# codex-storage/codex-storage-proofs-circuits

Hardware: AMD Instinct MI355X
Metric: Poseidon2-BN254 permutations/sec per GPU; full proof-input witnesses/sec (higher is better)
Workload: dtype u32x9 (29-bit limbs, Montgomery mod BN254 r)

## Files before the change

### codex-storage-proofs-circuits_amd/csrc/proof_many.cpp

```cpp
#include <hip/hip_runtime.h>

#include <algorithm>
#include <cstring>
#include <map>
#include <memory>
#include <string>
#include <vector>

#include "dataset_obj.hpp"
#include "proof_input_obj.hpp"
#include "trees.hpp"

using namespace cp2i;

namespace {

struct Req {
  cp2_dataset* ds = nullptr;
  uint64_t slot = 0;
  uint8_t entropy[32];
  size_t at = 0;
  size_t id = 0;
};

int refuse(cp2_ctx* ctx, size_t i, const std::string& why) {
  ctx->err = "request " + std::to_string(i) + ": " + why;
  return CP2_ERR_INVALID;
}

size_t depth_of(size_t n) { return layer_sizes_of(n).size() - 1; }

bool same_circuit(const cp2_config& a, const cp2_config& b) {
  return a.max_depth == b.max_depth && a.max_log2_nslots == b.max_log2_nslots && a.cell_size == b.cell_size && a.block_size == b.block_size &&
         a.n_samples == b.n_samples;
}

int validate(cp2_ctx* ctx, cp2_dataset* const* ds, const uint64_t* slot_idx, size_t n) {
  for (size_t i = 0; i < n; ++i) {
    const cp2_dataset* d = ds[i];
    if (!d) return refuse(ctx, i, "NULL dataset");
    if (d->ctx != ctx) return refuse(ctx, i, "its dataset belongs to another context");
    const cp2_config& c = d->cfg;
    if (!same_circuit(c, ds[0]->cfg))
      return refuse(ctx, i, "its circuit parameters (maxDepth, maxLog2NSlots, cellSize, blockSize, nSamples) differ from request 0's");
    const uint64_t s = slot_idx[i];
    if (s < d->first_slot || s - d->first_slot >= d->n_local)
      return refuse(ctx, i, "slot " + std::to_string(s) + " is not local to its dataset (slots " + std::to_string(d->first_slot) + " .. " +
                                std::to_string(d->first_slot + d->n_local - 1) + ")");
    if (!d->have_roots && !(d->first_slot == 0 && d->n_local == c.n_slots))
      return refuse(ctx, i, "its dataset has no dataset tree: not all of its slots are local and cp2_dataset_set_roots was never called");
    const std::string shape = proof_shape_refusal(c, config_slot_tree_depth(c), config_dataset_tree_depth(c));
    if (!shape.empty()) return refuse(ctx, i, shape);
    if (!d->trees && d->tree_mode == 2 && d->csizes.size() - 1 != depth_of(c.n_cells / (c.block_size / c.cell_size)))
      return refuse(ctx, i, "its compact layers do not match its configuration");
  }
  return CP2_OK;
}

int check_roots(cp2_ctx* ctx, cp2_dataset* const* ds, const uint64_t* slot_idx, size_t n) {
  std::vector<uint64_t> a(n);
  for (size_t i = 0; i < n; ++i)
    a[i] = (uint64_t)reinterpret_cast<uintptr_t>(dataset_roots_dev(ds[i])) + (slot_idx[i] - ds[i]->first_slot) * 32;
  std::vector<uint8_t> got(n * 32);
  DevBuf d_a, d_r;
  CP2_TRY(d_a.scratch(ctx, n * 8));
  CP2_TRY(d_r.scratch(ctx, n * 32));
  CP2_HIP(ctx, hipMemcpyAsync(d_a.p, a.data(), n * 8, hipMemcpyHostToDevice, ctx->stream));
  CP2_HIP(ctx, cp2k::launch_gather_addr(static_cast<const uint64_t*>(d_a.p), n, 32, d_r.p, ctx->stream));
  CP2_HIP(ctx, hipMemcpyAsync(got.data(), d_r.p, n * 32, hipMemcpyDeviceToHost, ctx->stream));
  CP2_HIP(ctx, hipStreamSynchronize(ctx->stream));
  for (size_t i = 0; i < n; ++i)
    if (std::memcmp(&got[i * 32], &ds[i]->dlayers[slot_idx[i] * 32], 32) != 0)
      return refuse(ctx, i, "the root its dataset tree holds for slot " + std::to_string(slot_idx[i]) +
                                " (cp2_dataset_set_roots) differs from the slot's built root");
  return CP2_OK;
}

int prepare(cp2_ctx* ctx, cp2_dataset* const* ds, const uint64_t* slot_idx, size_t n) {
  CP2_TRY(validate(ctx, ds, slot_idx, n));
  CP2_HIP(ctx, hipSetDevice(ctx->device));
  for (size_t i = 0; i < n; ++i)
    if (!ds[i]->have_roots) CP2_TRY(cp2_dataset_set_roots(ds[i], nullptr));
  return check_roots(ctx, ds, slot_idx, n);
}

std::string who(bool named, const Req* r) { return named ? "request " + std::to_string(r->id) + ": " : std::string(); }

int run_pass(cp2_ctx* ctx, const std::vector<const Req*>& rq, size_t n_rf, size_t n_rfile, size_t n_cf, bool named, cp2_proof_input** out) {
  const size_t n = rq.size(), nr = n_rf + n_rfile;
  const cp2_config& c0 = rq[0]->ds->cfg;
  const size_t ns = c0.n_samples, md = (size_t)c0.max_depth, cs = c0.cell_size, bs = c0.block_size, cpb = bs / cs;
  const size_t T = n * ns, R = nr * ns, C = T - R, RF = n_rf * ns, CF = n_cf * ns;
  auto store = std::make_shared<BatchStore>();
  if (T) {
    std::vector<cp2k::ManyReq> reqs(n);
    std::vector<cp2k::TreeGeom> geoms;
    std::map<std::string, uint32_t> geom_of;
    for (size_t j = 0; j < n; ++j) {
      const cp2_dataset* ds = rq[j]->ds;
      cp2k::ManyReq& q = reqs[j];
      std::memset(&q, 0, sizeof q);
      std::memcpy(q.entropy, rq[j]->entropy, 32);
      std::memcpy(q.slot_root, &ds->dlayers[rq[j]->slot * 32], 32);
      q.n_cells = ds->cfg.n_cells;
      q.cpb = cpb;
      if (j < nr) {
        cp2k::TreeGeom g;
        std::memset(&g, 0, sizeof g);
        trees_geom(ds->trees, &g);
        auto it = geom_of.emplace(std::string(reinterpret_cast<const char*>(&g), sizeof g), (uint32_t)geoms.size());
        if (it.second) geoms.push_back(g);
        q.geom = it.first->second;
        q.nodes = (uint64_t)reinterpret_cast<uintptr_t>(ds->trees->nodes.p);
        q.slot = rq[j]->slot - ds->first_slot;
      }
    }
    std::vector<uint64_t> blk(C), gen, cpaths, ctail, ccell;
    std::vector<uint8_t> checks(2 * C * 32);
    PinBuf h_blocks;
    const size_t rows = T * md + T + 2 * C;
    DevBuf d_req, d_geom, d_idx, d_blk, d_addr, d_rows, d_cells, d_gen, d_caddr;
    CP2_TRY(d_req.scratch(ctx, n * sizeof(cp2k::ManyReq)));
    CP2_TRY(d_geom.scratch(ctx, std::max<size_t>(1, geoms.size()) * sizeof(cp2k::TreeGeom)));
    CP2_TRY(d_idx.scratch(ctx, T * 8));
    CP2_TRY(d_blk.scratch(ctx, T * 8));
    CP2_TRY(d_addr.scratch(ctx, rows * 8));
    CP2_TRY(d_rows.scratch(ctx, rows * 32));
    CP2_TRY(d_cells.scratch(ctx, (C * cpb + T) * cs));
    CP2_TRY(store->idx.alloc(ctx, T * 8));
    CP2_TRY(store->paths.alloc(ctx, T * md * 32));
    CP2_TRY(store->leaves.alloc(ctx, T * 32));
    CP2_TRY(store->cells.alloc(ctx, T * cs));
    uint8_t* cells_out = d_cells.u8() + C * cpb * cs;
    uint64_t* addr = static_cast<uint64_t*>(d_addr.p);
    CP2_HIP(ctx, hipMemcpyAsync(d_req.p, reqs.data(), n * sizeof(cp2k::ManyReq), hipMemcpyHostToDevice, ctx->stream));
    if (!geoms.empty())
      CP2_HIP(ctx, hipMemcpyAsync(d_geom.p, geoms.data(), geoms.size() * sizeof(cp2k::TreeGeom), hipMemcpyHostToDevice, ctx->stream));
    CP2_HIP(ctx, cp2k::launch_sample_many(static_cast<const cp2k::ManyReq*>(d_req.p), static_cast<const cp2k::TreeGeom*>(d_geom.p), n,
                                          (uint32_t)ns, (uint32_t)md, static_cast<uint64_t*>(d_idx.p), static_cast<uint64_t*>(d_blk.p), addr,
                                          ctx->stream));
    CP2_HIP(ctx, hipMemcpyAsync(store->idx.p, d_idx.p, T * 8, hipMemcpyDeviceToHost, ctx->stream));
    if (C) CP2_HIP(ctx, hipMemcpyAsync(blk.data(), static_cast<uint64_t*>(d_blk.p) + R, C * 8, hipMemcpyDeviceToHost, ctx->stream));
    CP2_HIP(ctx, hipStreamSynchronize(ctx->stream));
    const uint64_t* idx = static_cast<const uint64_t*>(store->idx.p);

    gen.assign((CF + RF) * 2, 0);
    uint64_t* seeds = gen.data();
    uint64_t* firsts = seeds + CF + RF;
    for (size_t q = 0; q < CF; ++q) {
      const Req* r = rq[nr + q / ns];
      seeds[q] = cp2_slot_seed(r->ds->cfg.seed, r->slot);
      firsts[q] = blk[q] * cpb;
    }
    for (size_t p = 0; p < RF; ++p) {
      const Req* r = rq[p / ns];
      seeds[CF + p] = cp2_slot_seed(r->ds->cfg.seed, r->slot);
      firsts[CF + p] = idx[p];
    }
    if (CF + RF) {
      CP2_TRY(d_gen.scratch(ctx, gen.size() * 8));
      const uint64_t* dg = static_cast<const uint64_t*>(d_gen.p);
      CP2_HIP(ctx, hipMemcpyAsync(d_gen.p, gen.data(), gen.size() * 8, hipMemcpyHostToDevice, ctx->stream));
      CP2_HIP(ctx, cp2k::launch_gen_fake_cells_many(dg, dg + CF + RF, cpb, CF * cpb, cs, d_cells.p, ctx->stream));
      CP2_HIP(ctx, cp2k::launch_gen_fake_cells_many(dg + CF, dg + CF + RF + CF, 1, RF, cs, cells_out, ctx->stream));
    }
    if (C > CF) {
      const size_t n_req_file = (C - CF) / ns;
      CP2_TRY(h_blocks.alloc(ctx, (C - CF) * bs));
      std::vector<std::string> failed(fill_threads(ctx));
      on_threads(fill_threads(ctx), n_req_file, [&](int w, size_t k) {
        const size_t q0 = CF + k * ns;
        const Req* r = rq[nr + q0 / ns];
        const std::string fname = slot_file_name(r->ds->file_base, r->slot);
        size_t bad = 0;
        const int err = slot_file_read_list(fname, ns, [&](size_t) { return bs; }, [&](size_t c) { return blk[q0 + c] * bs; },
                                            [&](size_t c) { return h_blocks.u8() + (q0 - CF + c) * bs; }, &bad);
        if (err >= 0)
          failed[w] = who(named, r) + (err ? "block " + std::to_string(blk[q0 + bad]) + " of slot " : std::string("slot ")) + std::to_string(r->slot) +
                      ": " + slot_file_error(fname, err);
        return err < 0;
      });
      for (const auto& f : failed)
        if (!f.empty()) { ctx->err = f; return CP2_ERR_IO; }
      CP2_HIP(ctx, hipMemcpyAsync(d_cells.u8() + CF * bs, h_blocks.p, (C - CF) * bs, hipMemcpyHostToDevice, ctx->stream));
    }
    cp2_slot_trees* mini = nullptr;
    struct Mini { cp2_slot_trees*& t; ~Mini() { cp2_slot_trees_free(t); } } mini_guard{mini};
    if (C) {
      cpaths.assign(C * md, 0);
      ctail.assign(3 * C, 0);
      ccell.assign(C, 0);
      CP2_TRY(cp2_slot_trees_build_dev(ctx, d_cells.p, C, cs, bs, cpb, &mini));
      const size_t depth_b = depth_of(cpb);
      const uint64_t mb = (uint64_t)reinterpret_cast<uintptr_t>(mini->nodes.p);
      std::vector<uint64_t> rr(depth_b + 1);
      for (size_t q = 0; q < C; ++q) {
        const Req* r = rq[nr + q / ns];
        const cp2_dataset* ds = r->ds;
        const uint64_t ls = r->slot - ds->first_slot, cell = idx[R + q], b = blk[q], in_block = cell % cpb;
        const uint64_t kb = (uint64_t)reinterpret_cast<uintptr_t>(ds->compact.p);
        uint64_t* P = &cpaths[q * md];
        path_rows(mini, q, in_block, depth_b + 1, rr.data());
        for (size_t d = 0; d < depth_b; ++d) P[d] = rr[d] == NO_ROW ? 0 : mb + rr[d] * 32;
        uint64_t j = b, m = ds->cfg.n_cells / cpb;
        for (size_t d = 0; d + 1 < ds->csizes.size(); ++d) {
          const uint64_t sib = j ^ 1;
          P[depth_b + d] = sib < m ? kb + (ds->coff[d] + ls * ds->csizes[d] + sib) * 32 : 0;
          j >>= 1;
          m = (m + 1) >> 1;
        }
        ctail[q] = mb + (q * cpb + in_block) * 32;
        ctail[C + 2 * q] = kb + (ds->coff[0] + ls * ds->csizes[0] + b) * 32;
        ctail[C + 2 * q + 1] = mb + (mini->toff[0] + q) * 32;
        ccell[q] = (uint64_t)reinterpret_cast<uintptr_t>(d_cells.u8()) + (q * cpb + in_block) * cs;
      }
      CP2_TRY(d_caddr.scratch(ctx, C * 8));
      CP2_HIP(ctx, hipMemcpyAsync(addr + R * md, cpaths.data(), C * md * 8, hipMemcpyHostToDevice, ctx->stream));
      CP2_HIP(ctx, hipMemcpyAsync(addr + T * md + R, ctail.data(), 3 * C * 8, hipMemcpyHostToDevice, ctx->stream));
      CP2_HIP(ctx, hipMemcpyAsync(d_caddr.p, ccell.data(), C * 8, hipMemcpyHostToDevice, ctx->stream));
      CP2_HIP(ctx, cp2k::launch_gather_addr(static_cast<const uint64_t*>(d_caddr.p), C, cs, cells_out + R * cs, ctx->stream));
    }
    CP2_HIP(ctx, cp2k::launch_gather_addr(addr, rows, 32, d_rows.p, ctx->stream));
    CP2_HIP(ctx, hipMemcpyAsync(store->paths.p, d_rows.p, T * md * 32, hipMemcpyDeviceToHost, ctx->stream));
    CP2_HIP(ctx, hipMemcpyAsync(store->leaves.p, d_rows.u8() + T * md * 32, T * 32, hipMemcpyDeviceToHost, ctx->stream));
    if (C) CP2_HIP(ctx, hipMemcpyAsync(checks.data(), d_rows.u8() + (T * md + T) * 32, 2 * C * 32, hipMemcpyDeviceToHost, ctx->stream));
    CP2_HIP(ctx, hipMemcpyAsync(store->cells.p, cells_out, T * cs, hipMemcpyDeviceToHost, ctx->stream));
    CP2_HIP(ctx, hipStreamSynchronize(ctx->stream));
    for (size_t q = 0; q < C; ++q)
      if (std::memcmp(&checks[2 * q * 32], &checks[(2 * q + 1) * 32], 32) != 0) {
        const Req* r = rq[nr + q / ns];
        ctx->err = who(named, r) + "block " + std::to_string(blk[q]) + " of slot " + std::to_string(r->slot) +
                   " does not hash to its stored root (slot data changed since the build?)";
        return CP2_ERR_IO;
      }
    if (R > RF) {
      std::vector<std::string> failed(fill_threads(ctx));
      on_threads(fill_threads(ctx), n_rfile, [&](int w, size_t k) {
        const Req* r = rq[n_rf + k];
        const std::string fname = slot_file_name(r->ds->file_base, r->slot);
        const size_t p0 = (n_rf + k) * ns;
        const int err = slot_file_read_list(fname, ns, [&](size_t) { return cs; }, [&](size_t c) { return idx[p0 + c] * cs; },
                                            [&](size_t c) { return store->cells.u8() + (p0 + c) * cs; });
        if (err >= 0) failed[w] = who(named, r) + slot_file_error(fname, err);
        return err < 0;
      });
      for (const auto& f : failed)
        if (!f.empty()) { ctx->err = f; return CP2_ERR_IO; }
    }
  }
  std::vector<ProofItem> items(n);
  for (size_t j = 0; j < n; ++j) items[j] = {rq[j]->ds, rq[j]->slot, rq[j]->entropy, &out[rq[j]->at]};
  return proof_inputs_from_store(items.data(), n, store, store->cells.u8());
}

}

int cp2i::prove_requests(cp2_ctx* ctx, cp2_dataset* const* ds, const uint64_t* slot_idx, const uint8_t* entropies, size_t n, size_t at0,
                         bool named, cp2_proof_input** out) {
  for (size_t i = 0; i < n; ++i) out[i] = nullptr;
  if (n == 0) return CP2_OK;
  CP2_HIP(ctx, hipSetDevice(ctx->device));
  std::vector<Req> req(n);
  std::vector<const Req*> res_fake, res_file, cmp_fake, cmp_file, roots_only;
  for (size_t i = 0; i < n; ++i) {
    req[i].ds = ds[i];
    req[i].slot = slot_idx[i];
    req[i].at = i;
    req[i].id = at0 + i;
    canonical_felt(entropies + 32 * i, req[i].entropy);
    const cp2_dataset* d = ds[i];
    (d->trees ? (d->from_file ? res_file : res_fake) : d->tree_mode == 2 ? (d->from_file ? cmp_file : cmp_fake) : roots_only).push_back(&req[i]);
  }
  auto fail = [&](int st) {
    for (size_t i = 0; i < n; ++i) { cp2_proof_input_free(out[i]); out[i] = nullptr; }
    return st;
  };
  for (const Req* r : roots_only) {
    const int st = cp2_proof_inputs_generate_batch(r->ds, &r->slot, 1, r->entropy, &out[r->at]);
    if (st != CP2_OK) {
      ctx->err = who(named, r) + ctx->err;
      return fail(st);
    }
  }
  const cp2_config& c0 = ds[0]->cfg;
  const size_t per_req = std::max<size_t>(1, (size_t)c0.n_samples * c0.block_size);
  const size_t chunk = std::max<size_t>(1, ctx->stage_bytes / per_req);
  std::vector<const Req*> compact(cmp_fake);
  compact.insert(compact.end(), cmp_file.begin(), cmp_file.end());
  const size_t n_res = res_fake.size() + res_file.size();
  size_t c = 0;
  for (bool first = true; first ? n_res + compact.size() > 0 : c < compact.size(); first = false) {
    std::vector<const Req*> rq;
    if (first) {
      rq = res_fake;
      rq.insert(rq.end(), res_file.begin(), res_file.end());
    }
    const size_t c1 = std::min(compact.size(), c + chunk);
    rq.insert(rq.end(), compact.begin() + (long)c, compact.begin() + (long)c1);
    const size_t n_cf = c < cmp_fake.size() ? std::min(c1, cmp_fake.size()) - c : 0;
    const int st = run_pass(ctx, rq, first ? res_fake.size() : 0, first ? res_file.size() : 0, n_cf, named, out);
    if (st != CP2_OK) return fail(st);
    c = c1;
  }
  return CP2_OK;
}

extern "C" int cp2_proof_inputs_generate_many(cp2_ctx* ctx, cp2_dataset* const* ds, const uint64_t* slot_idx, const uint8_t* entropies, size_t n,
                                              cp2_proof_input** out) try {
  if (!ctx) return CP2_ERR_INVALID;
  if (n && (!ds || !slot_idx || !entropies || !out)) {
    ctx->err = "cp2_proof_inputs_generate_many: NULL array";
    return CP2_ERR_INVALID;
  }
  for (size_t i = 0; i < n; ++i) out[i] = nullptr;
  if (n == 0) return CP2_OK;
  CP2_REFUSE_STUCK(ctx);
  CP2_TRY(prepare(ctx, ds, slot_idx, n));
  return prove_requests(ctx, ds, slot_idx, entropies, n, 0, true, out);
} catch (const std::bad_alloc&) {
  return CP2_ERR_ALLOC;
} catch (...) {
  return CP2_ERR_INVALID;
}

extern "C" int cp2_proof_inputs_export_many(cp2_ctx* ctx, cp2_dataset* const* ds, const uint64_t* slot_idx, const uint8_t* entropies, size_t n,
                                            const char* const* paths, int threads, size_t batch, uint64_t* total_bytes) try {
  if (!ctx) return CP2_ERR_INVALID;
  if (n && (!ds || !slot_idx || !entropies)) {
    ctx->err = "cp2_proof_inputs_export_many: NULL array";
    return CP2_ERR_INVALID;
  }
  if (total_bytes) *total_bytes = 0;
  if (n == 0) return CP2_OK;
  CP2_REFUSE_STUCK(ctx);
  CP2_TRY(prepare(ctx, ds, slot_idx, n));
  return export_in_chunks(n, batch, threads, [&](size_t b0, size_t m, cp2_proof_input** out) {
    return prove_requests(ctx, ds + b0, slot_idx + b0, entropies + 32 * b0, m, b0, true, out);
  }, [&](size_t i) { return paths ? paths[i] : nullptr; }, total_bytes);
} catch (const std::bad_alloc&) {
  return CP2_ERR_ALLOC;
} catch (...) {
  return CP2_ERR_INVALID;
}
```

Measured before the change: 753.8 million.

## Deduplicate compact-mode blocks across requests with an up-front sampling pass plan

Compact-mode requests are now sampled on the GPU in one up-front pass. A hash-table planner then groups them into passes by the number of distinct (dataset, slot, block) triples rather than by request count. Each pass generates or reads, mini-tree-builds and root-checks only the distinct blocks, and lanes map back to them through an index table. This targets repeated block loads and hashing when samples or requests hit the same blocks. The cost is an extra sampling launch with a host sync and a host-side planning step, which gain nothing when blocks rarely repeat.

```diff
diff --git a/codex-storage-proofs-circuits_amd/csrc/proof_many.cpp b/codex-storage-proofs-circuits_amd/csrc/proof_many.cpp
--- a/codex-storage-proofs-circuits_amd/csrc/proof_many.cpp
+++ b/codex-storage-proofs-circuits_amd/csrc/proof_many.cpp
@@ -1,6 +1,8 @@
 #include <hip/hip_runtime.h>
 
 #include <algorithm>
+#include <cstdio>
+#include <cstdlib>
 #include <cstring>
 #include <map>
 #include <memory>
@@ -9,6 +11,7 @@
 
 #include "dataset_obj.hpp"
 #include "proof_input_obj.hpp"
+#include "proof_pass_plan.hpp"
 #include "trees.hpp"
 
 using namespace cp2i;
@@ -86,17 +89,55 @@
 
 std::string who(bool named, const Req* r) { return named ? "request " + std::to_string(r->id) + ": " : std::string(); }
 
-int run_pass(cp2_ctx* ctx, const std::vector<const Req*>& rq, size_t n_rf, size_t n_rfile, size_t n_cf, bool named, cp2_proof_input** out) {
+constexpr size_t SAMPLE_SLICE_LANES = (size_t)1 << 30;
+
+int sample_compact(cp2_ctx* ctx, const std::vector<const Req*>& rq, std::vector<uint64_t>& idx, std::vector<uint64_t>& blk) {
+  const size_t n = rq.size();
+  if (n == 0) return CP2_OK;
+  const cp2_config& c0 = rq[0]->ds->cfg;
+  const size_t ns = c0.n_samples, L = n * ns;
+  if (L == 0) return CP2_OK;
+  std::vector<cp2k::ManyReq> reqs(n);
+  for (size_t j = 0; j < n; ++j) {
+    const cp2_dataset* ds = rq[j]->ds;
+    cp2k::ManyReq& q = reqs[j];
+    std::memset(&q, 0, sizeof q);
+    std::memcpy(q.entropy, rq[j]->entropy, 32);
+    std::memcpy(q.slot_root, &ds->dlayers[rq[j]->slot * 32], 32);
+    q.n_cells = ds->cfg.n_cells;
+    q.cpb = c0.block_size / c0.cell_size;
+  }
+  idx.resize(L);
+  blk.resize(L);
+  DevBuf d_req, d_idx, d_blk;
+  CP2_TRY(d_req.scratch(ctx, n * sizeof(cp2k::ManyReq)));
+  CP2_TRY(d_idx.scratch(ctx, L * 8));
+  CP2_TRY(d_blk.scratch(ctx, L * 8));
+  CP2_HIP(ctx, hipMemcpyAsync(d_req.p, reqs.data(), n * sizeof(cp2k::ManyReq), hipMemcpyHostToDevice, ctx->stream));
+  const size_t per = std::max<size_t>(1, SAMPLE_SLICE_LANES / ns);
+  for (size_t r0 = 0; r0 < n; r0 += per)
+    CP2_HIP(ctx, cp2k::launch_sample_many(static_cast<const cp2k::ManyReq*>(d_req.p) + r0, nullptr, std::min(per, n - r0), (uint32_t)ns,
+                                          (uint32_t)c0.max_depth, static_cast<uint64_t*>(d_idx.p) + r0 * ns, static_cast<uint64_t*>(d_blk.p) + r0 * ns,
+                                          nullptr, ctx->stream));
+  CP2_HIP(ctx, hipMemcpyAsync(idx.data(), d_idx.p, L * 8, hipMemcpyDeviceToHost, ctx->stream));
+  CP2_HIP(ctx, hipMemcpyAsync(blk.data(), d_blk.p, L * 8, hipMemcpyDeviceToHost, ctx->stream));
+  CP2_HIP(ctx, hipStreamSynchronize(ctx->stream));
+  return CP2_OK;
+}
+
+int run_pass(cp2_ctx* ctx, const std::vector<const Req*>& rq, size_t n_rf, size_t n_rfile, size_t n_cf, const ProofPass* plan, const uint64_t* cidx,
+             bool named, cp2_proof_input** out) {
   const size_t n = rq.size(), nr = n_rf + n_rfile;
   const cp2_config& c0 = rq[0]->ds->cfg;
   const size_t ns = c0.n_samples, md = (size_t)c0.max_depth, cs = c0.cell_size, bs = c0.block_size, cpb = bs / cs;
-  const size_t T = n * ns, R = nr * ns, C = T - R, RF = n_rf * ns, CF = n_cf * ns;
+  const size_t T = n * ns, R = nr * ns, C = T - R, RF = n_rf * ns;
+  const size_t D = plan ? plan->n_distinct() : 0, DF = plan ? plan->n_fake : 0;
   auto store = std::make_shared<BatchStore>();
   if (T) {
-    std::vector<cp2k::ManyReq> reqs(n);
+    std::vector<cp2k::ManyReq> reqs(nr);
     std::vector<cp2k::TreeGeom> geoms;
     std::map<std::string, uint32_t> geom_of;
-    for (size_t j = 0; j < n; ++j) {
+    for (size_t j = 0; j < nr; ++j) {
       const cp2_dataset* ds = rq[j]->ds;
       cp2k::ManyReq& q = reqs[j];
       std::memset(&q, 0, sizeof q);
@@ -104,103 +145,110 @@
       std::memcpy(q.slot_root, &ds->dlayers[rq[j]->slot * 32], 32);
       q.n_cells = ds->cfg.n_cells;
       q.cpb = cpb;
-      if (j < nr) {
-        cp2k::TreeGeom g;
-        std::memset(&g, 0, sizeof g);
-        trees_geom(ds->trees, &g);
-        auto it = geom_of.emplace(std::string(reinterpret_cast<const char*>(&g), sizeof g), (uint32_t)geoms.size());
-        if (it.second) geoms.push_back(g);
-        q.geom = it.first->second;
-        q.nodes = (uint64_t)reinterpret_cast<uintptr_t>(ds->trees->nodes.p);
-        q.slot = rq[j]->slot - ds->first_slot;
-      }
-    }
-    std::vector<uint64_t> blk(C), gen, cpaths, ctail, ccell;
-    std::vector<uint8_t> checks(2 * C * 32);
+      cp2k::TreeGeom g;
+      std::memset(&g, 0, sizeof g);
+      trees_geom(ds->trees, &g);
+      auto it = geom_of.emplace(std::string(reinterpret_cast<const char*>(&g), sizeof g), (uint32_t)geoms.size());
+      if (it.second) geoms.push_back(g);
+      q.geom = it.first->second;
+      q.nodes = (uint64_t)reinterpret_cast<uintptr_t>(ds->trees->nodes.p);
+      q.slot = rq[j]->slot - ds->first_slot;
+    }
+    auto first_of = [&](size_t d) { return rq[nr + plan->first_lane[d] / ns]; };
+    std::vector<uint64_t> gen, cpaths, ctail, ccell;
+    std::vector<uint8_t> checks(2 * D * 32);
     PinBuf h_blocks;
-    const size_t rows = T * md + T + 2 * C;
-    DevBuf d_req, d_geom, d_idx, d_blk, d_addr, d_rows, d_cells, d_gen, d_caddr;
-    CP2_TRY(d_req.scratch(ctx, n * sizeof(cp2k::ManyReq)));
-    CP2_TRY(d_geom.scratch(ctx, std::max<size_t>(1, geoms.size()) * sizeof(cp2k::TreeGeom)));
-    CP2_TRY(d_idx.scratch(ctx, T * 8));
-    CP2_TRY(d_blk.scratch(ctx, T * 8));
+    const size_t rows = T * md + T + 2 * D;
+    DevBuf d_req, d_geom, d_idx, d_blk, d_raddr, d_addr, d_rows, d_cells, d_gen, d_caddr;
     CP2_TRY(d_addr.scratch(ctx, rows * 8));
     CP2_TRY(d_rows.scratch(ctx, rows * 32));
-    CP2_TRY(d_cells.scratch(ctx, (C * cpb + T) * cs));
+    CP2_TRY(d_cells.scratch(ctx, (D * cpb + T) * cs));
     CP2_TRY(store->idx.alloc(ctx, T * 8));
     CP2_TRY(store->paths.alloc(ctx, T * md * 32));
     CP2_TRY(store->leaves.alloc(ctx, T * 32));
     CP2_TRY(store->cells.alloc(ctx, T * cs));
-    uint8_t* cells_out = d_cells.u8() + C * cpb * cs;
+    uint8_t* cells_out = d_cells.u8() + D * cpb * cs;
     uint64_t* addr = static_cast<uint64_t*>(d_addr.p);
-    CP2_HIP(ctx, hipMemcpyAsync(d_req.p, reqs.data(), n * sizeof(cp2k::ManyReq), hipMemcpyHostToDevice, ctx->stream));
-    if (!geoms.empty())
+    uint64_t* idx = static_cast<uint64_t*>(store->idx.p);
+    if (C) std::memcpy(idx + R, cidx, C * 8);
+    if (R) {
+      CP2_TRY(d_req.scratch(ctx, nr * sizeof(cp2k::ManyReq)));
+      CP2_TRY(d_geom.scratch(ctx, geoms.size() * sizeof(cp2k::TreeGeom)));
+      CP2_TRY(d_idx.scratch(ctx, R * 8));
+      CP2_TRY(d_blk.scratch(ctx, R * 8));
+      if (C) CP2_TRY(d_raddr.scratch(ctx, (R * md + R) * 8));
+      uint64_t* raddr = C ? static_cast<uint64_t*>(d_raddr.p) : addr;
+      CP2_HIP(ctx, hipMemcpyAsync(d_req.p, reqs.data(), nr * sizeof(cp2k::ManyReq), hipMemcpyHostToDevice, ctx->stream));
       CP2_HIP(ctx, hipMemcpyAsync(d_geom.p, geoms.data(), geoms.size() * sizeof(cp2k::TreeGeom), hipMemcpyHostToDevice, ctx->stream));
-    CP2_HIP(ctx, cp2k::launch_sample_many(static_cast<const cp2k::ManyReq*>(d_req.p), static_cast<const cp2k::TreeGeom*>(d_geom.p), n,
-                                          (uint32_t)ns, (uint32_t)md, static_cast<uint64_t*>(d_idx.p), static_cast<uint64_t*>(d_blk.p), addr,
-                                          ctx->stream));
-    CP2_HIP(ctx, hipMemcpyAsync(store->idx.p, d_idx.p, T * 8, hipMemcpyDeviceToHost, ctx->stream));
-    if (C) CP2_HIP(ctx, hipMemcpyAsync(blk.data(), static_cast<uint64_t*>(d_blk.p) + R, C * 8, hipMemcpyDeviceToHost, ctx->stream));
-    CP2_HIP(ctx, hipStreamSynchronize(ctx->stream));
-    const uint64_t* idx = static_cast<const uint64_t*>(store->idx.p);
-
-    gen.assign((CF + RF) * 2, 0);
+      CP2_HIP(ctx, cp2k::launch_sample_many(static_cast<const cp2k::ManyReq*>(d_req.p), static_cast<const cp2k::TreeGeom*>(d_geom.p), nr,
+                                            (uint32_t)ns, (uint32_t)md, static_cast<uint64_t*>(d_idx.p), static_cast<uint64_t*>(d_blk.p), raddr,
+                                            ctx->stream));
+      if (C) {
+        if (md) CP2_HIP(ctx, hipMemcpyAsync(addr, raddr, R * md * 8, hipMemcpyDeviceToDevice, ctx->stream));
+        CP2_HIP(ctx, hipMemcpyAsync(addr + T * md, raddr + R * md, R * 8, hipMemcpyDeviceToDevice, ctx->stream));
+      }
+      CP2_HIP(ctx, hipMemcpyAsync(idx, d_idx.p, R * 8, hipMemcpyDeviceToHost, ctx->stream));
+      CP2_HIP(ctx, hipStreamSynchronize(ctx->stream));
+    }
+
+    gen.assign((DF + RF) * 2, 0);
     uint64_t* seeds = gen.data();
-    uint64_t* firsts = seeds + CF + RF;
-    for (size_t q = 0; q < CF; ++q) {
-      const Req* r = rq[nr + q / ns];
-      seeds[q] = cp2_slot_seed(r->ds->cfg.seed, r->slot);
-      firsts[q] = blk[q] * cpb;
+    uint64_t* firsts = seeds + DF + RF;
+    for (size_t d = 0; d < DF; ++d) {
+      const Req* r = first_of(d);
+      seeds[d] = cp2_slot_seed(r->ds->cfg.seed, r->slot);
+      firsts[d] = plan->block[d] * cpb;
     }
     for (size_t p = 0; p < RF; ++p) {
       const Req* r = rq[p / ns];
-      seeds[CF + p] = cp2_slot_seed(r->ds->cfg.seed, r->slot);
-      firsts[CF + p] = idx[p];
-    }
-    if (CF + RF) {
+      seeds[DF + p] = cp2_slot_seed(r->ds->cfg.seed, r->slot);
+      firsts[DF + p] = idx[p];
+    }
+    if (DF + RF) {
       CP2_TRY(d_gen.scratch(ctx, gen.size() * 8));
       const uint64_t* dg = static_cast<const uint64_t*>(d_gen.p);
       CP2_HIP(ctx, hipMemcpyAsync(d_gen.p, gen.data(), gen.size() * 8, hipMemcpyHostToDevice, ctx->stream));
-      CP2_HIP(ctx, cp2k::launch_gen_fake_cells_many(dg, dg + CF + RF, cpb, CF * cpb, cs, d_cells.p, ctx->stream));
-      CP2_HIP(ctx, cp2k::launch_gen_fake_cells_many(dg + CF, dg + CF + RF + CF, 1, RF, cs, cells_out, ctx->stream));
-    }
-    if (C > CF) {
-      const size_t n_req_file = (C - CF) / ns;
-      CP2_TRY(h_blocks.alloc(ctx, (C - CF) * bs));
+      CP2_HIP(ctx, cp2k::launch_gen_fake_cells_many(dg, dg + DF + RF, cpb, DF * cpb, cs, d_cells.p, ctx->stream));
+      CP2_HIP(ctx, cp2k::launch_gen_fake_cells_many(dg + DF, dg + DF + RF + DF, 1, RF, cs, cells_out, ctx->stream));
+    }
+    if (D > DF) {
+      CP2_TRY(h_blocks.alloc(ctx, (D - DF) * bs));
       std::vector<std::string> failed(fill_threads(ctx));
-      on_threads(fill_threads(ctx), n_req_file, [&](int w, size_t k) {
-        const size_t q0 = CF + k * ns;
-        const Req* r = rq[nr + q0 / ns];
+      on_threads(fill_threads(ctx), plan->n_requests() - n_cf, [&](int w, size_t kf) {
+        const size_t k = n_cf + kf, d0 = plan->own[k], d1 = plan->own[k + 1];
+        if (d0 == d1) return true;
+        const Req* r = rq[nr + k];
         const std::string fname = slot_file_name(r->ds->file_base, r->slot);
         size_t bad = 0;
-        const int err = slot_file_read_list(fname, ns, [&](size_t) { return bs; }, [&](size_t c) { return blk[q0 + c] * bs; },
-                                            [&](size_t c) { return h_blocks.u8() + (q0 - CF + c) * bs; }, &bad);
+        const int err = slot_file_read_list(fname, d1 - d0, [&](size_t) { return bs; }, [&](size_t c) { return plan->block[d0 + c] * bs; },
+                                            [&](size_t c) { return h_blocks.u8() + (d0 - DF + c) * bs; }, &bad);
         if (err >= 0)
-          failed[w] = who(named, r) + (err ? "block " + std::to_string(blk[q0 + bad]) + " of slot " : std::string("slot ")) + std::to_string(r->slot) +
-                      ": " + slot_file_error(fname, err);
+          failed[w] = who(named, r) + (err ? "block " + std::to_string(plan->block[d0 + bad]) + " of slot " : std::string("slot ")) +
+                      std::to_string(r->slot) + ": " + slot_file_error(fname, err);
         return err < 0;
       });
       for (const auto& f : failed)
         if (!f.empty()) { ctx->err = f; return CP2_ERR_IO; }
-      CP2_HIP(ctx, hipMemcpyAsync(d_cells.u8() + CF * bs, h_blocks.p, (C - CF) * bs, hipMemcpyHostToDevice, ctx->stream));
+      CP2_HIP(ctx, hipMemcpyAsync(d_cells.u8() + DF * bs, h_blocks.p, (D - DF) * bs, hipMemcpyHostToDevice, ctx->stream));
     }
     cp2_slot_trees* mini = nullptr;
     struct Mini { cp2_slot_trees*& t; ~Mini() { cp2_slot_trees_free(t); } } mini_guard{mini};
     if (C) {
       cpaths.assign(C * md, 0);
-      ctail.assign(3 * C, 0);
+      ctail.assign(C + 2 * D, 0);
       ccell.assign(C, 0);
-      CP2_TRY(cp2_slot_trees_build_dev(ctx, d_cells.p, C, cs, bs, cpb, &mini));
+      CP2_TRY(cp2_slot_trees_build_dev(ctx, d_cells.p, D, cs, bs, cpb, &mini));
       const size_t depth_b = depth_of(cpb);
       const uint64_t mb = (uint64_t)reinterpret_cast<uintptr_t>(mini->nodes.p);
       std::vector<uint64_t> rr(depth_b + 1);
       for (size_t q = 0; q < C; ++q) {
         const Req* r = rq[nr + q / ns];
         const cp2_dataset* ds = r->ds;
-        const uint64_t ls = r->slot - ds->first_slot, cell = idx[R + q], b = blk[q], in_block = cell % cpb;
+        const size_t dd = plan->of_lane[q];
+        const uint64_t ls = r->slot - ds->first_slot, cell = idx[R + q], b = plan->block[dd], in_block = cell % cpb;
         const uint64_t kb = (uint64_t)reinterpret_cast<uintptr_t>(ds->compact.p);
         uint64_t* P = &cpaths[q * md];
-        path_rows(mini, q, in_block, depth_b + 1, rr.data());
+        path_rows(mini, dd, in_block, depth_b + 1, rr.data());
         for (size_t d = 0; d < depth_b; ++d) P[d] = rr[d] == NO_ROW ? 0 : mb + rr[d] * 32;
         uint64_t j = b, m = ds->cfg.n_cells / cpb;
         for (size_t d = 0; d + 1 < ds->csizes.size(); ++d) {
@@ -209,27 +257,32 @@
           j >>= 1;
           m = (m + 1) >> 1;
         }
-        ctail[q] = mb + (q * cpb + in_block) * 32;
-        ctail[C + 2 * q] = kb + (ds->coff[0] + ls * ds->csizes[0] + b) * 32;
-        ctail[C + 2 * q + 1] = mb + (mini->toff[0] + q) * 32;
-        ccell[q] = (uint64_t)reinterpret_cast<uintptr_t>(d_cells.u8()) + (q * cpb + in_block) * cs;
+        ctail[q] = mb + (dd * cpb + in_block) * 32;
+        ccell[q] = (uint64_t)reinterpret_cast<uintptr_t>(d_cells.u8()) + (dd * cpb + in_block) * cs;
+      }
+      for (size_t d = 0; d < D; ++d) {
+        const Req* r = first_of(d);
+        const cp2_dataset* ds = r->ds;
+        const uint64_t kb = (uint64_t)reinterpret_cast<uintptr_t>(ds->compact.p), ls = r->slot - ds->first_slot;
+        ctail[C + 2 * d] = kb + (ds->coff[0] + ls * ds->csizes[0] + plan->block[d]) * 32;
+        ctail[C + 2 * d + 1] = mb + (mini->toff[0] + d) * 32;
       }
       CP2_TRY(d_caddr.scratch(ctx, C * 8));
       CP2_HIP(ctx, hipMemcpyAsync(addr + R * md, cpaths.data(), C * md * 8, hipMemcpyHostToDevice, ctx->stream));
-      CP2_HIP(ctx, hipMemcpyAsync(addr + T * md + R, ctail.data(), 3 * C * 8, hipMemcpyHostToDevice, ctx->stream));
+      CP2_HIP(ctx, hipMemcpyAsync(addr + T * md + R, ctail.data(), ctail.size() * 8, hipMemcpyHostToDevice, ctx->stream));
       CP2_HIP(ctx, hipMemcpyAsync(d_caddr.p, ccell.data(), C * 8, hipMemcpyHostToDevice, ctx->stream));
       CP2_HIP(ctx, cp2k::launch_gather_addr(static_cast<const uint64_t*>(d_caddr.p), C, cs, cells_out + R * cs, ctx->stream));
     }
     CP2_HIP(ctx, cp2k::launch_gather_addr(addr, rows, 32, d_rows.p, ctx->stream));
     CP2_HIP(ctx, hipMemcpyAsync(store->paths.p, d_rows.p, T * md * 32, hipMemcpyDeviceToHost, ctx->stream));
     CP2_HIP(ctx, hipMemcpyAsync(store->leaves.p, d_rows.u8() + T * md * 32, T * 32, hipMemcpyDeviceToHost, ctx->stream));
-    if (C) CP2_HIP(ctx, hipMemcpyAsync(checks.data(), d_rows.u8() + (T * md + T) * 32, 2 * C * 32, hipMemcpyDeviceToHost, ctx->stream));
+    if (D) CP2_HIP(ctx, hipMemcpyAsync(checks.data(), d_rows.u8() + (T * md + T) * 32, 2 * D * 32, hipMemcpyDeviceToHost, ctx->stream));
     CP2_HIP(ctx, hipMemcpyAsync(store->cells.p, cells_out, T * cs, hipMemcpyDeviceToHost, ctx->stream));
     CP2_HIP(ctx, hipStreamSynchronize(ctx->stream));
-    for (size_t q = 0; q < C; ++q)
-      if (std::memcmp(&checks[2 * q * 32], &checks[(2 * q + 1) * 32], 32) != 0) {
-        const Req* r = rq[nr + q / ns];
-        ctx->err = who(named, r) + "block " + std::to_string(blk[q]) + " of slot " + std::to_string(r->slot) +
+    for (size_t d = 0; d < D; ++d)
+      if (std::memcmp(&checks[2 * d * 32], &checks[(2 * d + 1) * 32], 32) != 0) {
+        const Req* r = first_of(d);
+        ctx->err = who(named, r) + "block " + std::to_string(plan->block[d]) + " of slot " + std::to_string(r->slot) +
                    " does not hash to its stored root (slot data changed since the build?)";
         return CP2_ERR_IO;
       }
@@ -283,24 +336,37 @@
     }
   }
   const cp2_config& c0 = ds[0]->cfg;
-  const size_t per_req = std::max<size_t>(1, (size_t)c0.n_samples * c0.block_size);
-  const size_t chunk = std::max<size_t>(1, ctx->stage_bytes / per_req);
+  const size_t ns = c0.n_samples;
   std::vector<const Req*> compact(cmp_fake);
   compact.insert(compact.end(), cmp_file.begin(), cmp_file.end());
+  std::vector<uint64_t> cidx, cblk;
+  const int sampled = sample_compact(ctx, compact, cidx, cblk);
+  if (sampled != CP2_OK) return fail(sampled);
+  std::vector<PassIdentity> ident(compact.size());
+  for (size_t j = 0; j < compact.size(); ++j) ident[j] = {(uint64_t)reinterpret_cast<uintptr_t>(compact[j]->ds), compact[j]->slot};
+  const std::vector<ProofPass> plan = proof_pass_plan(ident.data(), cblk.data(), compact.size(), cmp_fake.size(), ns, c0.block_size, ctx->stage_bytes);
+  if (std::getenv("CP2_TRACE") && !plan.empty()) {
+    size_t distinct = 0;
+    for (const ProofPass& p : plan) distinct += p.n_distinct();
+    std::fprintf(stderr, "[cp2 trace] compact proof inputs: %zu request(s) in %zu pass(es), %zu distinct block(s) of %zu touched\n", compact.size(),
+                 plan.size(), distinct, compact.size() * ns);
+  }
   const size_t n_res = res_fake.size() + res_file.size();
-  size_t c = 0;
-  for (bool first = true; first ? n_res + compact.size() > 0 : c < compact.size(); first = false) {
+  for (size_t k = 0; k < std::max<size_t>(plan.size(), n_res ? 1 : 0); ++k) {
+    const bool first = k == 0;
+    const ProofPass* p = k < plan.size() ? &plan[k] : nullptr;
     std::vector<const Req*> rq;
     if (first) {
       rq = res_fake;
       rq.insert(rq.end(), res_file.begin(), res_file.end());
     }
-    const size_t c1 = std::min(compact.size(), c + chunk);
-    rq.insert(rq.end(), compact.begin() + (long)c, compact.begin() + (long)c1);
-    const size_t n_cf = c < cmp_fake.size() ? std::min(c1, cmp_fake.size()) - c : 0;
-    const int st = run_pass(ctx, rq, first ? res_fake.size() : 0, first ? res_file.size() : 0, n_cf, named, out);
+    size_t n_cf = 0;
+    if (p) {
+      rq.insert(rq.end(), compact.begin() + (long)p->r0, compact.begin() + (long)p->r1);
+      n_cf = std::min(std::max(cmp_fake.size(), p->r0), p->r1) - p->r0;
+    }
+    const int st = run_pass(ctx, rq, first ? res_fake.size() : 0, first ? res_file.size() : 0, n_cf, p, p ? cidx.data() + p->r0 * ns : nullptr, named, out);
     if (st != CP2_OK) return fail(st);
-    c = c1;
   }
   return CP2_OK;
 }
diff --git a/codex-storage-proofs-circuits_amd/csrc/proof_pass_plan.hpp b/codex-storage-proofs-circuits_amd/csrc/proof_pass_plan.hpp
--- /dev/null
+++ b/codex-storage-proofs-circuits_amd/csrc/proof_pass_plan.hpp
@@ -0,0 +1,81 @@
+#pragma once
+#include <algorithm>
+#include <cstddef>
+#include <cstdint>
+#include <vector>
+
+namespace cp2i {
+
+struct PassIdentity {
+  uint64_t object = 0, slot = 0;
+};
+
+struct ProofPass {
+  size_t r0 = 0, r1 = 0;
+  std::vector<uint64_t> block;
+  std::vector<size_t> first_lane;
+  std::vector<size_t> of_lane;
+  std::vector<size_t> own;
+  size_t n_fake = 0;
+  size_t n_requests() const { return r1 - r0; }
+  size_t n_distinct() const { return block.size(); }
+};
+
+inline std::vector<ProofPass> proof_pass_plan(const PassIdentity* ident, const uint64_t* blocks, size_t n_req, size_t n_fake_req,
+                                              size_t n_samples, size_t block_size, size_t stage_bytes) {
+  std::vector<ProofPass> passes;
+  if (n_req == 0) return passes;
+  const size_t ns = n_samples, lanes = n_req * ns;
+  const size_t cap = stage_bytes / std::max<size_t>(1, block_size);
+  struct Entry {
+    uint64_t object, slot, block;
+    size_t index, stamp;
+  };
+  const size_t most = cap >= lanes ? lanes : std::min(lanes, cap + ns);
+  size_t mask = 15;
+  while (mask + 1 < 2 * most) mask = 2 * mask + 1;
+  std::vector<Entry> table(mask + 1, Entry{0, 0, 0, 0, 0});
+  size_t stamp = 0, r = 0;
+  while (r < n_req) {
+    passes.emplace_back();
+    ProofPass& p = passes.back();
+    p.r0 = r;
+    p.own.push_back(0);
+    ++stamp;
+    for (; r < n_req; ++r) {
+      const size_t blocks_before = p.block.size(), lanes_before = p.of_lane.size();
+      const PassIdentity& id = ident[r];
+      for (size_t c = 0; c < ns; ++c) {
+        const uint64_t b = blocks[r * ns + c];
+        uint64_t h = (id.object + 0x9e3779b97f4a7c15ULL) * 0xbf58476d1ce4e5b9ULL ^ (id.slot + 0x632be59bd9b4e019ULL) * 0x94d049bb133111ebULL ^
+                     b * 0xd6e8feb86659fd93ULL;
+        h ^= h >> 32;
+        size_t at = (size_t)h & mask;
+        while (table[at].stamp == stamp && !(table[at].block == b && table[at].slot == id.slot && table[at].object == id.object))
+          at = (at + 1) & mask;
+        if (table[at].stamp != stamp) {
+          table[at] = Entry{id.object, id.slot, b, p.block.size(), stamp};
+          p.block.push_back(b);
+          p.first_lane.push_back(lanes_before + c);
+        }
+        p.of_lane.push_back(table[at].index);
+      }
+      if (p.block.size() > cap && r > p.r0) {
+        p.block.resize(blocks_before);
+        p.first_lane.resize(blocks_before);
+        p.of_lane.resize(lanes_before);
+        break;
+      }
+      p.own.push_back(p.block.size());
+      if (p.block.size() > cap) {
+        ++r;
+        break;
+      }
+    }
+    p.r1 = r;
+    p.n_fake = p.own[std::min(std::max(n_fake_req, p.r0), p.r1) - p.r0];
+  }
+  return passes;
+}
+
+}
```

Result: no change. 755.2 million (median of 2 runs) (+0.2%).
